# dusk-network/schnorr

Measured on AMD Instinct MI355X. Metric: Schnorr verifies/sec (single + double) at batch=2^20; 1/2/4/8 MI355X, higher is better.
Workload: dtype u32x9 (29-bit limbs, u64 accumulate); 1 GPU; 2^20 single-signature batch verify per GPU (BASELINE configs[1]); `value` is this figure, `double` / `vargen` / `mixed` ride along with --full; batch_per_gpu=1048576, parallelism=dp1, collective=none

## Files before the change

### schnorr_amd/csrc/common.h

```cpp
#pragma once
#include <hip/hip_runtime.h>

#include "fe29.h"
#include "fr.h"
#include "jubjub29.h"
#include "launch.h"

namespace dsv {

static_assert(kLimbs == NL, "launch.h and fe29.h disagree on the limb count");

constexpr int kFixedHalf = 1 << (kFixedBits - 1);

DSV_DEV void load_words8(u32 (&w)[8], const uint8_t* base, size_t idx) {
  const uint4* p = reinterpret_cast<const uint4*>(base + idx * 32);
  uint4 a = p[0], b = p[1];
  w[0] = a.x; w[1] = a.y; w[2] = a.z; w[3] = a.w;
  w[4] = b.x; w[5] = b.y; w[6] = b.z; w[7] = b.w;
}
DSV_DEV void store_words8(uint8_t* base, size_t idx, const u32 (&w)[8]) {
  uint4* p = reinterpret_cast<uint4*>(base + idx * 32);
  p[0] = make_uint4(w[0], w[1], w[2], w[3]);
  p[1] = make_uint4(w[4], w[5], w[6], w[7]);
}
DSV_DEV bool load_fq(Fe& out, const uint8_t* base, size_t idx) {
  u32 w[8];
  load_words8(w, base, idx);
  bool ok = words_lt(w, kQ32);
  out = fe_to_mont(fe_from_words_plain(w));
  return ok;
}
DSV_DEV bool load_fq_signed(Fe& out, const uint8_t* base, size_t idx, bool negate) {
  u32 w[8];
  load_words8(w, base, idx);
  const bool ok = words_lt(w, kQ32);
  u32 borrow = 0;
#pragma unroll
  for (int i = 0; i < 8; i++) {
    const u64 t = (u64)kQ32[i] - w[i] - borrow;
    borrow = (u32)(t >> 63);
    w[i] = negate ? (u32)t : w[i];
  }
  out = fe_to_mont(fe_from_words_plain(w));
  return ok;
}
DSV_DEV void store_fq(uint8_t* base, size_t idx, const Fe& mont) {
  u32 w[8];
  fe_to_words_plain(w, fe_from_mont(mont));
  store_words8(base, idx, w);
}

DSV_DEV ANiels load_aniels(const u32* __restrict__ table, int window, int d) {
  const bool neg = d < 0;
  const u32 mag = (u32)(neg ? -d : d);
  const u32* p = table + ((size_t)window * kFixedEntries + mag) * kEntryWords;
  ANiels n;
#pragma unroll
  for (int i = 0; i < NL; i++) {
    n.vpu.l[i] = p[(neg ? NL : 0) + i];
    n.vmu.l[i] = p[(neg ? 0 : NL) + i];
    n.t2d.l[i] = p[(neg ? 3 * NL : 2 * NL) + i];
  }
  return n;
}

DSV_DEV void recode_fixed(u32 (&y)[9], const u32 (&s)[8]) {
  u32 carry = 0;
#pragma unroll
  for (int i = 0; i < 9; i++) {
    u32 bias = 0;
#pragma unroll
    for (int k = 0; k < kFixedWindows; k++) {
      const int pos = kFixedBits * k + kFixedBits - 1;
      if ((pos >> 5) == i) bias |= 1u << (pos & 31);
    }
    const u64 t = (u64)(i < 8 ? s[i] : 0u) + bias + carry;
    y[i] = (u32)t;
    carry = (u32)(t >> 32);
  }
}
DSV_DEV int next_fixed_digit(u32 (&y)[9]) {
  const int d = (int)(y[0] & ((1u << kFixedBits) - 1)) - kFixedHalf;
#pragma unroll
  for (int i = 0; i < 8; i++) y[i] = __funnelshift_r(y[i], y[i + 1], kFixedBits);
  y[8] >>= kFixedBits;
  return d;
}
DSV_DEV Ext fixed_base_accumulate(Ext acc, const u32 (&s)[8], const u32* __restrict__ table) {
  u32 y[9];
  recode_fixed(y, s);
#pragma unroll 1
  for (int w = 0; w < kFixedWindows; w++) {
    const int d = next_fixed_digit(y);
    ANiels e = load_aniels(table, w, d);
    acc = ext_add_aniels(acc, e);
  }
  return acc;
}

DSV_DEV bool fixed_base_accumulate_is_identity(Ext acc, const u32 (&s)[8], const u32* __restrict__ table) {
  u32 y[9];
  recode_fixed(y, s);
#pragma unroll 1
  for (int w = 0; w < kFixedWindows - 1; w++) {
    const int d = next_fixed_digit(y);
    ANiels e = load_aniels(table, w, d);
    acc = ext_add_aniels(acc, e);
  }
  return ext_add_aniels_is_identity(acc, load_aniels(table, kFixedWindows - 1, next_fixed_digit(y)));
}

DSV_DEV void store_fe_words(u32* p, const Fe& a) {
#pragma unroll
  for (int i = 0; i < NL; i++) p[i] = a.l[i];
}
DSV_DEV Fe load_fe_words(const u32* p) {
  Fe r;
#pragma unroll
  for (int i = 0; i < NL; i++) r.l[i] = p[i];
  return r;
}
DSV_DEV void store_var_entry(u32* lane_tbl, int e, const Niels& n) {
  u32* p = lane_tbl + e * kVarEntryWords;
  store_fe_words(p, n.vpu);
  store_fe_words(p + NL, n.vmu);
  store_fe_words(p + 2 * NL, n.z);
  store_fe_words(p + 3 * NL, n.t2d);
}
__device__ const u32 kIdentityEntry[4 * NL] = {
    DSV_ONE_LIST, DSV_ONE_LIST, DSV_ONE_LIST, 0, 0, 0, 0, 0, 0, 0, 0, 0};
DSV_DEV Niels load_var_entry(const u32* lane_tbl, int d) {
  const bool neg = d < 0;
  const int mag = neg ? -d : d;
  const u32* p = mag == 0 ? kIdentityEntry : lane_tbl + mag * kVarEntryWords;
  Niels n;
  n.vpu = load_fe_words(p + (neg ? NL : 0));
  n.vmu = load_fe_words(p + (neg ? 0 : NL));
  n.z = load_fe_words(p + 2 * NL);
  const Fe t = load_fe_words(p + 3 * NL);
  n.t2d = fe_select(neg, fe_neg2(t), t);
  return n;
}
struct RawNiels {
  Fe a, b, z, t;
  bool neg;
};
DSV_DEV RawNiels load_var_entry_raw(const u32* lane_tbl, int d) {
  RawNiels r;
  r.neg = d < 0;
  const int mag = r.neg ? -d : d;
  const u32* p = mag == 0 ? kIdentityEntry : lane_tbl + mag * kVarEntryWords;
  r.a = load_fe_words(p + (r.neg ? NL : 0));
  r.b = load_fe_words(p + (r.neg ? 0 : NL));
  r.z = load_fe_words(p + 2 * NL);
  r.t = load_fe_words(p + 3 * NL);
  return r;
}
DSV_DEV Niels finish_var_entry(const RawNiels& r) {
  Niels n;
  n.vpu = r.a;
  n.vmu = r.b;
  n.z = r.z;
  n.t2d = fe_select(r.neg, fe_neg2(r.t), r.t);
  return n;
}
DSV_DEV void build_var_table(u32* lane_tbl, const Fe& pu, const Fe& pv) {
  Ext p = ext_from_affine(pu, pv);
  Fe tt = fe_mul(p.t1, p.t2);
  Niels n1 = ext_to_niels_t(p, tt);
  store_var_entry(lane_tbl, 1, n1);
  const ANiels a1 = {n1.vpu, n1.vmu, n1.t2d};
  Ext cur = p;
#pragma unroll 1
  for (int i = 2; i < kVarEntries; i++) {
    cur = ext_add_aniels_t(cur, tt, a1);
    tt = fe_mul(cur.t1, cur.t2);
    store_var_entry(lane_tbl, i, ext_to_niels_t(cur, tt));
  }
}
DSV_DEV void recode_signed4(u32 (&y)[8], const u32 (&s)[8]) {
  u32 carry = 0;
#pragma unroll
  for (int i = 0; i < 8; i++) {
    u64 t = (u64)s[i] + 0x88888888u + carry;
    y[i] = (u32)t;
    carry = (u32)(t >> 32);
  }
}
DSV_DEV int sdigit4(const u32 (&y)[8], int k) {
  return (int)((y[k >> 3] >> (4 * (k & 7))) & 0xf) - 8;
}
DSV_DEV int top_digit4(const u32 (&nz)[8]) {
  int len = 0;
#pragma unroll
  for (int i = 0; i < 8; i++)
    if (nz[i] != 0) len = 32 * i + (32 - __clz(nz[i]));
  return len > 0 ? (len - 1) >> 2 : 0;
}

constexpr int kJointSlots = 12;
constexpr int kJointLaneWords = kJointSlots * kVarEntryWords;
static_assert(kJointLaneWords <= 2 * kVarLaneWords, "the joint table lives in the two one-base slots");
DSV_DEV int joint_slot(u32 ra, u32 rb) {
  const u32 idx = ra * 4 + rb;
  const unsigned long long slots = 0xB73895164202A615ULL;
  const int slot = (int)((slots >> (4 * idx)) & 15u);
  const bool neg = ((0x17u >> idx) & 1u) != 0;
  return neg ? -slot : slot;
}
DSV_DEV void recode_signed2(u32 (&y)[8], const u32 (&s)[8]) {
  u32 carry = 0;
#pragma unroll
  for (int i = 0; i < 8; i++) {
    const u64 t = (u64)s[i] + 0x55555555u + carry;
    y[i] = (u32)t;
    carry = (u32)(t >> 32);
  }
}
DSV_DEV int joint_digit(const u32 (&ya)[8], const u32 (&yb)[8], int k) {
  const int sh = 2 * (k & 15);
  return joint_slot((ya[k >> 4] >> sh) & 3u, (yb[k >> 4] >> sh) & 3u);
}
DSV_DEV int top_digit2(const u32 (&nz)[8]) {
  int len = 0;
#pragma unroll
  for (int i = 0; i < 8; i++)
    if (nz[i] != 0) len = 32 * i + (32 - __clz(nz[i]));
  return len > 0 ? (len - 1) >> 1 : 0;
}
DSV_DEV void build_joint_table(u32* tbl, const Fe& pu, const Fe& pv, const Fe& ru, const Fe& rv) {
  const Ext P = ext_from_affine(pu, pv), R = ext_from_affine(ru, rv);
  const Fe ttP = fe_mul(pu, pv), ttR = fe_mul(ru, rv);
  const Niels nP = ext_to_niels_t(P, ttP), nR = ext_to_niels_t(R, ttR);
  store_var_entry(tbl, 1, nP);
  store_var_entry(tbl, 2, nR);
  const ANiels aR = {nR.vpu, nR.vmu, nR.t2d};
  auto put = [&](int slot, const Ext& x) { store_var_entry(tbl, slot, ext_to_niels(x)); };
  Ext sum, diff;
  {
    ext_add_sub_aniels_t(sum, diff, P, ttP, aR);
    put(5, sum);
    put(6, diff);
    put(11, ext_double(sum));
  }
  {
    const Ext P2 = ext_double_affine(pu, pv);
    const Fe tt = fe_mul(P2.t1, P2.t2);
    store_var_entry(tbl, 3, ext_to_niels_t(P2, tt));
    ext_add_sub_aniels_t(sum, diff, P2, tt, aR);
    put(7, sum);
    put(8, diff);
  }
  {
    const Ext R2 = ext_double_affine(ru, rv);
    const Fe tt = fe_mul(R2.t1, R2.t2);
    store_var_entry(tbl, 4, ext_to_niels_t(R2, tt));
    const u32* e1 = tbl + 1 * kVarEntryWords;
    const ANiels aP = {load_fe_words(e1), load_fe_words(e1 + NL), load_fe_words(e1 + 3 * NL)};
    ext_add_sub_aniels_t(sum, diff, R2, tt, aP);
    put(9, sum);
    put(10, diff);
  }
}
DSV_DEV Ext ext_mul4(const Ext& p) {
  Ext q = p;
  ext_double_uvz(q.u, q.v, q.z);
  return ext_double(q);
}

DSV_DEV Ext ext_mul16(const Ext& p) {
  Fe u = p.u, v = p.v, z = p.z;
#pragma unroll 1
  for (int j = 0; j < 3; j++) ext_double_uvz(u, v, z);
  Ext q;
  q.u = u;
  q.v = v;
  q.z = z;
  return ext_double(q);
}

template <int TOP>
DSV_DEV Ext var_base_mul(const u32 (&s)[8], const u32* lane_tbl) {
  u32 y[8];
  recode_signed4(y, s);
  Ext acc = ext_from_niels(load_var_entry(lane_tbl, sdigit4(y, TOP)));
#pragma unroll 1
  for (int k = TOP - 1; k >= 0; k--) {
    acc = ext_mul16(acc);
    acc = ext_add_niels(acc, load_var_entry(lane_tbl, sdigit4(y, k)));
  }
  return acc;
}

DSV_DEV void store_poison(uint8_t* base, size_t idx) {
  const u32 w[8] = {~0u, ~0u, ~0u, ~0u, ~0u, ~0u, ~0u, ~0u};
  store_words8(base, idx, w);
}

}
```

### schnorr_amd/csrc/fr.h

```cpp
#pragma once
#include "fe29.h"

namespace dsv {

__device__ constexpr u32 kFrR2[8] = {0x95e57731u, 0x67719aa4u, 0x9ce3fc26u, 0x51b0cef0u,
                                     0xc026e9a5u, 0x69dab7fau, 0x8d127688u, 0x04f6547bu};
constexpr u32 kFrInv32 = 0xef788ef9u;

DSV_DEV void fr_mont_mul(u32 (&out)[8], const u32 (&a)[8], const u32 (&b)[8]) {
  u32 t[10];
#pragma unroll
  for (int i = 0; i < 10; i++) t[i] = 0;
#pragma unroll 1
  for (int i = 0; i < 8; i++) {
    u64 c = 0;
#pragma unroll
    for (int j = 0; j < 8; j++) {
      u64 x = (u64)a[j] * b[i] + t[j] + c;
      t[j] = (u32)x;
      c = x >> 32;
    }
    u64 x = (u64)t[8] + c;
    t[8] = (u32)x;
    t[9] = (u32)(x >> 32);
    u32 m = t[0] * kFrInv32;
    c = ((u64)m * kR32[0] + t[0]) >> 32;
#pragma unroll
    for (int j = 1; j < 8; j++) {
      u64 y = (u64)m * kR32[j] + t[j] + c;
      t[j - 1] = (u32)y;
      c = y >> 32;
    }
    x = (u64)t[8] + c;
    t[7] = (u32)x;
    t[8] = t[9] + (u32)(x >> 32);
  }
  u32 d[8];
  u32 borrow = 0;
#pragma unroll
  for (int j = 0; j < 8; j++) {
    u64 y = (u64)t[j] - kR32[j] - borrow;
    d[j] = (u32)y;
    borrow = (u32)(y >> 63);
  }
  const bool ge = (t[8] != 0) | (borrow == 0);
#pragma unroll
  for (int j = 0; j < 8; j++) out[j] = ge ? d[j] : t[j];
}
DSV_DEV void fr_mul(u32 (&out)[8], const u32 (&a)[8], const u32 (&b)[8]) {
  u32 t[8];
  fr_mont_mul(t, a, b);
  fr_mont_mul(out, t, kFrR2);
}
DSV_DEV void fr_sub(u32 (&out)[8], const u32 (&a)[8], const u32 (&b)[8]) {
  u32 d[8];
  u32 borrow = 0;
#pragma unroll
  for (int j = 0; j < 8; j++) {
    u64 y = (u64)a[j] - b[j] - borrow;
    d[j] = (u32)y;
    borrow = (u32)(y >> 63);
  }
  u32 carry = 0;
#pragma unroll
  for (int j = 0; j < 8; j++) {
    u64 y = (u64)d[j] + (borrow ? kR32[j] : 0u) + carry;
    out[j] = (u32)y;
    carry = (u32)(y >> 32);
  }
}

}
```

### schnorr_amd/csrc/k_verify.hip

```cpp
#include "common.h"
#include "halfgcd.h"

namespace dsv {

template <int NCHAIN>
__global__ void __launch_bounds__(kVerifyBlock, kWavesVerify)
k_verify_fixed_half(const uint8_t* __restrict__ u, const uint8_t* __restrict__ c, ChainOperands op0,
                    ChainOperands op1, const uint8_t* __restrict__ valid, bool accumulate, size_t n,
                    uint8_t* __restrict__ ok, u32* __restrict__ var_tables, const u32* __restrict__ gate) {
  if (gate_says_done(gate)) return;
  u32* tbl = var_tables + ((size_t)blockIdx.x * kVerifyBlock + threadIdx.x) * kJointLaneWords;
#pragma unroll 1
  for (size_t base = (size_t)blockIdx.x * kVerifyBlock; base < n;
       base += (size_t)gridDim.x * kVerifyBlock) {
    const size_t i = base + threadIdx.x;
    if (i >= n) continue;
    bool good = accumulate ? (ok[i] != 0) : (valid[i] != 0);
    u32 ya[8], yb[8], w[8];
    bool b_neg;
    int top;
    {
      u32 cs[8], a[8], b[8];
      load_words8(cs, c, i);
      half_scalars(a, b, b_neg, cs);
      recode_signed2(ya, a);
      recode_signed2(yb, b);
      u32 nz[8];
#pragma unroll
      for (int k = 0; k < 8; k++) nz[k] = (ya[k] ^ 0x55555555u) | (yb[k] ^ 0x55555555u);
      top = top_digit2(nz);
      u32 us[8];
      load_words8(us, u, i);
      const bool u_ok = words_lt(us, kR32);
      good &= u_ok;
      if (!u_ok) us[7] &= 0x0fffffffu;
      fr_mul(w, b, us);
      if (b_neg) {
        const u32 zero[8] = {0, 0, 0, 0, 0, 0, 0, 0};
        u32 t[8];
        fr_sub(t, zero, w);
#pragma unroll
        for (int k = 0; k < 8; k++) w[k] = t[k];
      }
    }
#pragma unroll 1
    for (int h = 0; h < NCHAIN; h++) {
      const ChainOperands op = h ? op1 : op0;
      {
        Fe pku, pkv, ru, rv;
        good &= load_fq(pku, op.PK_uv, 2 * i);
        good &= load_fq(pkv, op.PK_uv, 2 * i + 1);
        good &= load_fq_signed(ru, op.R_uv, 2 * i, !b_neg);
        good &= load_fq(rv, op.R_uv, 2 * i + 1);
        build_joint_table(tbl, pku, pkv, ru, rv);
      }
      Ext acc = ext_from_niels(load_var_entry(tbl, joint_digit(ya, yb, top)));
      {
        RawNiels e = load_var_entry_raw(tbl, joint_digit(ya, yb, top > 0 ? top - 1 : 0));
#pragma unroll 1
        for (int k = top - 1; k >= 0; k--) {
          acc = ext_mul4(acc);
          const Niels cur = finish_var_entry(e);
          e = load_var_entry_raw(tbl, joint_digit(ya, yb, k > 0 ? k - 1 : 0));
          acc = ext_add_niels(acc, cur);
        }
      }
      good &= fixed_base_accumulate_is_identity(acc, w, op.table);
    }
    ok[i] = good ? 1 : 0;
  }
}

void launch_verify_half(int nchain, bool accumulate, const uint8_t* u, const uint8_t* c,
                        ChainOperands op0, ChainOperands op1, const uint8_t* valid, size_t n,
                        uint8_t* ok, uint32_t* var_tables, hipStream_t s, const uint32_t* gate) {
  const dim3 grid(verify_grid(n)), block(kVerifyBlock);
  if (nchain == 2)
    hipLaunchKernelGGL(k_verify_fixed_half<2>, grid, block, 0, s, u, c, op0, op1, valid, accumulate, n,
                       ok, var_tables, gate);
  else
    hipLaunchKernelGGL(k_verify_fixed_half<1>, grid, block, 0, s, u, c, op0, op1, valid, accumulate, n,
                       ok, var_tables, gate);
}

}
```

Measured before the change: 83.66 million verifies/s.

## Use wave-uniform digit loop, spill recoded scalars to table, shorten scalar mul

The recoded joint scalars are stored into the per-lane table scratch and read back one word at a time, which frees 16 live registers in the main loop. The loop bound becomes the wave-wide maximum top digit, so all lanes run the same trip count instead of diverging per lane. fr_mul is replaced by a CIOS multiply that uses only the 5 low words of the half-size scalar b. The Niels addition is also inlined so the next table load is issued between the multiplies. The costs are extra scratch memory traffic and extra leading doublings for lanes whose scalars are shorter than the wave maximum.

New measurement: 84.06 million verifies/s, median of 5. Within noise of the previous version (+0.5%).

```diff
diff --git a/schnorr_amd/csrc/common.h b/schnorr_amd/csrc/common.h
--- a/schnorr_amd/csrc/common.h
+++ b/schnorr_amd/csrc/common.h
@@ -161,7 +161,8 @@
   n.vpu = r.a;
   n.vmu = r.b;
   n.z = r.z;
-  n.t2d = fe_select(r.neg, fe_neg2(r.t), r.t);
+#pragma unroll
+  for (int i = 0; i < NL; i++) n.t2d.l[i] = r.neg ? kBias2[i] - r.t.l[i] : r.t.l[i];
   return n;
 }
 DSV_DEV void build_var_table(u32* lane_tbl, const Fe& pu, const Fe& pv) {
@@ -217,10 +218,6 @@
     carry = (u32)(t >> 32);
   }
 }
-DSV_DEV int joint_digit(const u32 (&ya)[8], const u32 (&yb)[8], int k) {
-  const int sh = 2 * (k & 15);
-  return joint_slot((ya[k >> 4] >> sh) & 3u, (yb[k >> 4] >> sh) & 3u);
-}
 DSV_DEV int top_digit2(const u32 (&nz)[8]) {
   int len = 0;
 #pragma unroll
@@ -228,6 +225,54 @@
     if (nz[i] != 0) len = 32 * i + (32 - __clz(nz[i]));
   return len > 0 ? (len - 1) >> 1 : 0;
 }
+DSV_DEV int wave_max7(int v) {
+  int m = 0;
+  bool cand = true;
+#pragma unroll
+  for (int bit = 6; bit >= 0; bit--) {
+    const bool has = cand && ((v >> bit) & 1) != 0;
+    const bool any = __builtin_amdgcn_ballot_w64(has) != 0;
+    m |= (int)any << bit;
+    cand = any ? has : cand;
+  }
+  return __builtin_amdgcn_readfirstlane(m);
+}
+DSV_DEV void store_joint_scalars(u32* tbl, const u32 (&ya)[8], const u32 (&yb)[8]) {
+  uint4* p = reinterpret_cast<uint4*>(tbl);
+  p[0] = make_uint4(ya[0], ya[1], ya[2], ya[3]);
+  p[1] = make_uint4(ya[4], ya[5], ya[6], ya[7]);
+  p[2] = make_uint4(yb[0], yb[1], yb[2], yb[3]);
+  p[3] = make_uint4(yb[4], yb[5], yb[6], yb[7]);
+}
+struct JointDigits {
+  u32 wa, wb;
+  u32 na, nb;
+};
+DSV_DEV void joint_digits_ahead(JointDigits& d, const u32* tbl, int w) {
+  const int wn = w > 0 ? w - 1 : 0;
+  d.na = tbl[wn];
+  d.nb = tbl[8 + wn];
+}
+DSV_DEV JointDigits joint_digits_begin(const u32* tbl, int k) {
+  JointDigits d;
+  d.wa = tbl[k >> 4];
+  d.wb = tbl[8 + (k >> 4)];
+  joint_digits_ahead(d, tbl, k >> 4);
+  return d;
+}
+DSV_DEV int joint_digit_here(const JointDigits& d, int k) {
+  const u32 sh = 2u * ((u32)k & 15u);
+  return joint_slot(__builtin_amdgcn_ubfe(d.wa, sh, 2u), __builtin_amdgcn_ubfe(d.wb, sh, 2u));
+}
+DSV_DEV int joint_digit_walk(JointDigits& d, const u32* tbl, int k) {
+  if ((k & 15) == 15) {
+    d.wa = d.na;
+    d.wb = d.nb;
+    joint_digits_ahead(d, tbl, k >> 4);
+  }
+  return joint_digit_here(d, k);
+}
+
 DSV_DEV void build_joint_table(u32* tbl, const Fe& pu, const Fe& pv, const Fe& ru, const Fe& rv) {
   const Ext P = ext_from_affine(pu, pv), R = ext_from_affine(ru, rv);
   const Fe ttP = fe_mul(pu, pv), ttR = fe_mul(ru, rv);
diff --git a/schnorr_amd/csrc/fr.h b/schnorr_amd/csrc/fr.h
--- a/schnorr_amd/csrc/fr.h
+++ b/schnorr_amd/csrc/fr.h
@@ -52,6 +52,64 @@
   fr_mont_mul(t, a, b);
   fr_mont_mul(out, t, kFrR2);
 }
+__device__ constexpr u32 kFrR416[8] = {0xfa4f2421u, 0x6148df31u, 0xba4a71e5u, 0x1f9d3336u,
+                                       0xb025f946u, 0x28c5e2fbu, 0xb1953583u, 0x0277d41cu};
+DSV_DEV void fr_cios_round(u32 (&t)[9], const u32 (&a)[8], u32 bi) {
+  u64 c = 0;
+#pragma unroll
+  for (int j = 0; j < 8; j++) {
+    const u64 x = (u64)a[j] * bi + t[j] + c;
+    t[j] = (u32)x;
+    c = x >> 32;
+  }
+  u64 x = (u64)t[8] + c;
+  t[8] = (u32)x;
+  const u32 t9 = (u32)(x >> 32);
+  const u32 m = t[0] * kFrInv32;
+  c = ((u64)m * kR32[0] + t[0]) >> 32;
+#pragma unroll
+  for (int j = 1; j < 8; j++) {
+    const u64 y = (u64)m * kR32[j] + t[j] + c;
+    t[j - 1] = (u32)y;
+    c = y >> 32;
+  }
+  x = (u64)t[8] + c;
+  t[7] = (u32)x;
+  t[8] = t9 + (u32)(x >> 32);
+}
+DSV_DEV void fr_mul_short(u32 (&out)[8], const u32 (&b)[8], const u32 (&u)[8]) {
+  u32 t[9];
+#pragma unroll
+  for (int i = 0; i < 9; i++) t[i] = 0;
+  u32 w0 = b[0], w1 = b[1], w2 = b[2], w3 = b[3], w4 = b[4];
+#pragma unroll 1
+  for (int i = 0; i < 5; i++) {
+    fr_cios_round(t, u, w0);
+    w0 = w1;
+    w1 = w2;
+    w2 = w3;
+    w3 = w4;
+  }
+  u32 a[8];
+#pragma unroll
+  for (int i = 0; i < 8; i++) a[i] = t[i];
+#pragma unroll
+  for (int i = 0; i < 9; i++) t[i] = 0;
+#pragma unroll 1
+  for (int i = 0; i < 8; i++) fr_cios_round(t, a, kFrR416[i]);
+  u32 d[8];
+  u32 borrow = 0;
+#pragma unroll
+  for (int j = 0; j < 8; j++) {
+    const u64 y = (u64)t[j] - kR32[j] - borrow;
+    d[j] = (u32)y;
+    borrow = (u32)(y >> 63);
+  }
+  const bool ge = (t[8] != 0) | (borrow == 0);
+#pragma unroll
+  for (int j = 0; j < 8; j++) out[j] = ge ? d[j] : t[j];
+}
+
 DSV_DEV void fr_sub(u32 (&out)[8], const u32 (&a)[8], const u32 (&b)[8]) {
   u32 d[8];
   u32 borrow = 0;
diff --git a/schnorr_amd/csrc/k_verify.hip b/schnorr_amd/csrc/k_verify.hip
--- a/schnorr_amd/csrc/k_verify.hip
+++ b/schnorr_amd/csrc/k_verify.hip
@@ -16,15 +16,16 @@
     const size_t i = base + threadIdx.x;
     if (i >= n) continue;
     bool good = accumulate ? (ok[i] != 0) : (valid[i] != 0);
-    u32 ya[8], yb[8], w[8];
+    u32 w[8];
     bool b_neg;
     int top;
     {
-      u32 cs[8], a[8], b[8];
+      u32 cs[8], a[8], b[8], ya[8], yb[8];
       load_words8(cs, c, i);
       half_scalars(a, b, b_neg, cs);
       recode_signed2(ya, a);
       recode_signed2(yb, b);
+      store_joint_scalars(tbl, ya, yb);
       u32 nz[8];
 #pragma unroll
       for (int k = 0; k < 8; k++) nz[k] = (ya[k] ^ 0x55555555u) | (yb[k] ^ 0x55555555u);
@@ -34,7 +35,7 @@
       const bool u_ok = words_lt(us, kR32);
       good &= u_ok;
       if (!u_ok) us[7] &= 0x0fffffffu;
-      fr_mul(w, b, us);
+      fr_mul_short(w, b, us);
       if (b_neg) {
         const u32 zero[8] = {0, 0, 0, 0, 0, 0, 0, 0};
         u32 t[8];
@@ -43,6 +44,7 @@
         for (int k = 0; k < 8; k++) w[k] = t[k];
       }
     }
+    const int wtop = wave_max7(top);
 #pragma unroll 1
     for (int h = 0; h < NCHAIN; h++) {
       const ChainOperands op = h ? op1 : op0;
@@ -54,15 +56,20 @@
         good &= load_fq(rv, op.R_uv, 2 * i + 1);
         build_joint_table(tbl, pku, pkv, ru, rv);
       }
-      Ext acc = ext_from_niels(load_var_entry(tbl, joint_digit(ya, yb, top)));
+      JointDigits dg = joint_digits_begin(tbl, wtop);
+      Ext acc = ext_from_niels(load_var_entry(tbl, joint_digit_here(dg, wtop)));
       {
-        RawNiels e = load_var_entry_raw(tbl, joint_digit(ya, yb, top > 0 ? top - 1 : 0));
+        RawNiels e = load_var_entry_raw(tbl, joint_digit_walk(dg, tbl, wtop > 0 ? wtop - 1 : 0));
 #pragma unroll 1
-        for (int k = top - 1; k >= 0; k--) {
+        for (int k = wtop - 1; k >= 0; k--) {
           acc = ext_mul4(acc);
           const Niels cur = finish_var_entry(e);
-          e = load_var_entry_raw(tbl, joint_digit(ya, yb, k > 0 ? k - 1 : 0));
-          acc = ext_add_niels(acc, cur);
+          const Fe a = fe_mul(fe_sub2_raw(acc.v, acc.u), cur.vmu);
+          const Fe b = fe_mul(fe_add(acc.v, acc.u), cur.vpu);
+          const Fe c = fe_mul(fe_mul(acc.t1, acc.t2), cur.t2d);
+          const Fe d = fe_dbl(fe_mul(acc.z, cur.z));
+          e = load_var_entry_raw(tbl, joint_digit_walk(dg, tbl, k > 0 ? k - 1 : 0));
+          acc = ext_add_tail(a, b, c, d);
         }
       }
       good &= fixed_base_accumulate_is_identity(acc, w, op.table);
```
